# AIM-SE/AC-TSR

Measured on AMD Instinct MI355X. Metric: user-sequences/sec fwd+bwd, AC-SASRec L=50 d=64, 1/2/4/8 MI355X, higher is better.
Workload: dtype f32; 1 GPU; ACSASRec full training step (spatial + adversarial calibrators, BASELINE configs[2]), synthetic 100000-item catalogue, B=512/GPU L=50 d=64 h=2 2 layers inner=256, CE loss, two-pass backward + Adam; global_batch=512, seq_len=50, hidden=64, heads=2, parallelism=dp1, launch=hipGraph replay per step, backward=two walks (reference protocol, trainer.py:672-686)

## Files before the change

ac_tsr_amd/_lib.py:

```python
from __future__ import annotations

import ctypes as C
import os
import subprocess

_HERE = os.path.dirname(os.path.abspath(__file__))
CSRC = os.path.join(_HERE, "csrc")
LIB_PATH = os.environ.get("ACATTN_LIB") or os.path.join(CSRC, "libacattn.so")
HEADER_PATH = os.path.join(os.path.dirname(_HERE), "include", "acattn.h")

ABI_VERSION = 30
MAX_MASKS = 8
NSTAT = 8
MASK_STRUCTURED, MASK_DENSE_LL, MASK_DENSE_L = 0, 1, 2
COMBINE = {"fixed": 0, "gate": 1, "annealing": 2}
RICH = {"none": 0, "fixed": 1, "trainable": 2}
RNG_EXPLICIT, RNG_COUNTER = 0, 1
FWD_AUTO, FWD_STREAM, FWD_STAGED, FWD_GENERAL = 0, 1, 2, 3
BWD_AUTO, BWD_STREAM, BWD_ROW = 0, 1, 2

_f = C.c_void_p


class Problem(C.Structure):
    _fields_ = [
        ("B", C.c_int32), ("L", C.c_int32), ("H", C.c_int32), ("n_heads", C.c_int32),
# ... 60 lines not shown

ADAM_MAX_TENSORS = 64


class AdamGroup(C.Structure):
    _fields_ = [("n_tensors", C.c_int32), ("param", _f * ADAM_MAX_TENSORS), ("grad", _f * ADAM_MAX_TENSORS),
                ("exp_avg", _f * ADAM_MAX_TENSORS), ("exp_avg_sq", _f * ADAM_MAX_TENSORS), ("step", _f * ADAM_MAX_TENSORS),
                ("numel", C.c_int64 * ADAM_MAX_TENSORS)]


class TailProblem(C.Structure):
    _fields_ = [("rows", C.c_int32), ("H", C.c_int32), ("I", C.c_int32), ("ctx", _f), ("x", _f), ("wd", _f), ("bd", _f),
                ("g1", _f), ("b1", _f), ("w1", _f), ("bb1", _f), ("w2", _f), ("bb2", _f), ("g2", _f), ("b2", _f),
                ("eps1", C.c_float), ("eps2", C.c_float), ("p1", C.c_float), ("p2", C.c_float), ("keep1", _f),
                ("keep2", _f), ("seed1", C.c_uint64), ("seed2", C.c_uint64), ("seed_device", _f), ("src_index", _f),
                ("src_R", C.c_int32), ("src_L", C.c_int32)]


class TailSaved(C.Structure):
    _fields_ = [("h1", _f), ("st1", _f), ("a", _f), ("act", _f), ("h3", _f), ("st2", _f), ("out", _f),
                ("gelu_grad", _f)]


class TailBwdIO(C.Structure):
    _fields_ = [("d_out", _f), ("d_ctx", _f), ("d_x", _f), ("d_h1", _f), ("d_h2", _f), ("d_h3", _f), ("dgb_part", _f),
                ("workspace", _f)]


class EmbedProblem(C.Structure):
    _fields_ = [("rows", C.c_int32), ("L", C.c_int32), ("H", C.c_int32), ("n_table_rows", C.c_int64), ("idx", _f),
                ("table", _f), ("pos", _f), ("gamma", _f), ("beta", _f), ("eps", C.c_float), ("p_drop", C.c_float),
# ... 24 lines not shown
    "acattn_dropout_add_layernorm_fwd": (C.c_int, [C.POINTER(LnProblem), _f, _f, C.c_void_p]),
    "acattn_dropout_add_layernorm_bwd": (C.c_int, [C.POINTER(LnProblem), _f, _f, _f, _f, _f, C.c_void_p]),
    "acattn_embed_layernorm_fwd": (C.c_int, [C.POINTER(EmbedProblem), _f, _f, C.c_void_p]),
    "acattn_embed_layernorm_bwd": (C.c_int, [C.POINTER(EmbedProblem), _f, _f, C.c_int64, _f, _f, _f, C.c_void_p]),
    "acattn_projections_supported": (C.c_int, [C.c_int32, C.c_int32]),
    "acattn_projections_bwd_workspace_bytes": (C.c_int64, [C.POINTER(ProjProblem)]),
    "acattn_projections_fwd": (C.c_int, [C.POINTER(ProjProblem), C.POINTER(ProjOut), C.c_void_p]),
    "acattn_projections_bwd": (C.c_int, [C.POINTER(ProjProblem), C.POINTER(ProjBwdIO), C.c_void_p]),
    "acattn_layer_tail_supported": (C.c_int, [C.c_int32, C.c_int32]),
    "acattn_layer_tail_fwd": (C.c_int, [C.POINTER(TailProblem), C.POINTER(TailSaved), C.c_void_p]),
    "acattn_layer_tail_bwd": (C.c_int, [C.POINTER(TailProblem), C.POINTER(TailSaved), C.POINTER(TailBwdIO), C.c_void_p]),
    "acattn_layer_tail_bwd_partial_rows": (C.c_int32, [C.c_int32]),
    "acattn_layer_tail_bwd_partial_rows_for": (C.c_int32, [C.c_int32, C.c_int32]),
    "acattn_layer_tail_bwd_workspace_bytes": (C.c_int64, [C.c_int32, C.c_int32]),
    "acattn_select_layer_tail_blocks": (C.c_int, [C.c_int]),
    "acattn_adam_step": (C.c_int, [C.POINTER(AdamGroup), C.c_double, C.c_double, C.c_double, C.c_double, C.c_double, _f,
                                   C.c_void_p]),
    "acattn_dense_ce_fwd": (C.c_int, [_f, C.c_int64, C.c_int64, _f, _f, _f, C.c_void_p]),
    "acattn_dense_ce_bwd": (C.c_int, [_f, _f, _f, _f, C.c_int64, C.c_int64, _f, C.c_void_p]),
    "acattn_step_inputs": (C.c_int, [C.POINTER(C.c_void_p), C.POINTER(C.c_void_p), C.POINTER(C.c_int64), C.c_int32, C.c_void_p,
                                     C.c_void_p, C.c_void_p, C.c_int32, C.c_void_p]),
    "acattn_sum_rows": (C.c_int, [_f, _f, C.c_int32, C.c_int32, C.c_int32, C.c_void_p]),
    "acattn_sum_rows_pair": (C.c_int, [_f, _f, C.c_int32, C.c_int32, C.c_int32, _f, _f, C.c_int32, C.c_int32, C.c_int32, C.c_void_p]),
    "acattn_mask_penalty_fwd": (C.c_int, [_f, C.c_int64, _f, _f, C.c_void_p]),
    "acattn_mask_penalty_partial": (C.c_int, [_f, C.c_int64, _f, C.c_void_p]),
    "acattn_mask_penalty_partial_multi": (C.c_int, [C.c_void_p, C.c_int32, C.c_int64, _f, C.c_void_p]),
    "acattn_mask_penalty_bwd_scaled_multi": (C.c_int, [C.c_void_p, _f, _f, C.c_float, C.c_int64, C.c_void_p, C.c_int32,
                                                       C.c_void_p]),
    "acattn_attacked_loss_finish": (C.c_int, [_f, C.c_int32, _f, C.c_int32, C.c_int64, C.c_float, _f, _f, C.c_int32,
                                              C.c_void_p]),
# ... 68 lines not shown
```

ac_tsr_amd/csrc/acattn_api.hip:

```cpp
#include <stdint.h>
#include <stdio.h>
#include <string.h>

#include <algorithm>

#include "acattn_common.h"

namespace {
thread_local char g_err[256] = "";

int fail(const char* msg) {
  snprintf(g_err, sizeof(g_err), "%s", msg);
  return -1;
}

int check_problem(const acattn_problem* p) {
  if (!p) return fail("problem is NULL");
  if (p->B < 1 || p->L < 1 || p->H < 1 || p->n_heads < 1) return fail("B, L, H, n_heads must be positive");
  if (p->H % p->n_heads != 0)
    return fail("The hidden size is not a multiple of the number of attention heads");
  const int dh = p->H / p->n_heads;
  if (dh != 16 && dh != 32 && dh != 64 && dh != 128) return fail("unsupported head size: dh must be 16, 32, 64 or 128");
  if (p->L > 208) return fail("unsupported sequence length: L must be <= 208");
  if (!p->q || !p->k || !p->v) return fail("q, k, v must be non-NULL");
// ... 223 lines not shown
  if (!io->dmq_total && !io->dmk_total && !io->dx) return fail("projections backward: nothing to compute");
  const int rc = acattn_launch_proj_bwd(*p, *io, (hipStream_t)stream);
  if (rc > 0) snprintf(g_err, sizeof(g_err), "HIP launch failed: %s", hipGetErrorString((hipError_t)rc));
  return rc;
}

static int check_tail(const acattn_tail_problem* p, const acattn_tail_saved* s) {
  if (!p || !s) return fail("problem and saved must be non-NULL");
  if (p->rows < 1) return fail("rows must be positive");
  if (!acattn_tail_supported(p->H, p->I)) return fail("layer tail: (hidden_size, inner_size) must be (64, 256), (64, 128), (128, 512), (128, 256) or (256, 1024)");
  if (!p->ctx || !p->x || !p->wd || !p->bd || !p->g1 || !p->b1 || !p->w1 || !p->bb1 || !p->w2 || !p->bb2 || !p->g2 || !p->b2)
    return fail("layer tail: inputs and parameters must be non-NULL");
  if (!(p->p1 >= 0.f && p->p1 < 1.f) || !(p->p2 >= 0.f && p->p2 < 1.f)) return fail("dropout probabilities must be in [0, 1)");
  if (!s->h1 || !s->st1 || !s->a || !s->h3 || !s->st2) return fail("layer tail: saved tensors must be non-NULL");
  if (p->src_index && (p->src_R < 1 || p->src_L < 1)) return fail("layer tail: src_index needs src_R, src_L >= 1");
  return 0;
}

int acattn_layer_tail_supported(int32_t H, int32_t I) { return acattn_tail_supported(H, I) ? 1 : 0; }

int32_t acattn_layer_tail_bwd_partial_rows(int32_t rows) { return acattn_tail_bwd_partial_rows(rows); }
int32_t acattn_layer_tail_bwd_partial_rows_for(int32_t rows, int32_t H) { return acattn_tail_bwd_partial_rows_h(rows, H); }
int64_t acattn_layer_tail_bwd_workspace_bytes(int32_t H, int32_t I) {
  return acattn_tail_supported(H, I) ? acattn_tail_bwd_ws_bytes(H, I) : -1;
}

int acattn_select_layer_tail_blocks(int nb) {
  if (nb < 0 || nb > 2) return fail("rows per wave: 0 (automatic), 1 or 2 blocks of 16");
  return acattn_select_tail_nb(nb);
}

int acattn_layer_tail_fwd(const acattn_tail_problem* p, const acattn_tail_saved* saved, void* stream) {
  if (int rc = check_tail(p, saved)) return rc;
  if (!saved->act || !saved->out) return fail("layer tail forward: act and out must be non-NULL");
  const int rc = acattn_launch_tail_fwd(*p, *saved, (hipStream_t)stream);
  if (rc > 0) snprintf(g_err, sizeof(g_err), "HIP launch failed: %s", hipGetErrorString((hipError_t)rc));
  return rc;
}

// ... 295 lines not shown
```

ac_tsr_amd/csrc/acattn_common.h:

```cpp
#pragma once
#include <hip/hip_runtime.h>
#include <stdint.h>

#include <type_traits>

#include "acattn.h"

typedef float f4 __attribute__((ext_vector_type(4)));
typedef float f4u __attribute__((ext_vector_type(4), aligned(4)));

#define ACATTN_NEG_INF (-__builtin_inff())
#define ACATTN_MASK_FILL (-10000.0f)
#define ACATTN_LOG_EPS (1e-24f)

__device__ __forceinline__ float quad_sum(float x) {
  auto r = __builtin_amdgcn_permlane16_swap(__float_as_uint(x), __float_as_uint(x), false, false);
  x = __uint_as_float(r[0]) + __uint_as_float(r[1]);
  auto s = __builtin_amdgcn_permlane32_swap(__float_as_uint(x), __float_as_uint(x), false, false);
  return __uint_as_float(s[0]) + __uint_as_float(s[1]);
}

__device__ __forceinline__ float quad_max(float x) {
  auto r = __builtin_amdgcn_permlane16_swap(__float_as_uint(x), __float_as_uint(x), false, false);
  x = fmaxf(__uint_as_float(r[0]), __uint_as_float(r[1]));
// ... 249 lines not shown
int acattn_launch_ln_bwd(const acattn_ln_problem& p, const float* dy, const float* stats, float* dz, float* dres,
                         float* dgb_part, hipStream_t stream);
int acattn_launch_sum_rows(const float* x, float* out, int batch, int R, int C, hipStream_t stream);
int acattn_launch_sum_rows_pair(const float* x1, float* out1, int batch1, int R1, int C1, const float* x2, float* out2,
                                int batch2, int R2, int C2, hipStream_t stream);
void acattn_set_error(const char* msg);
bool acattn_proj_supported(int H, int G);
int64_t acattn_proj_bwd_ws_bytes(const acattn_proj_problem& p);
int acattn_launch_proj_fwd(const acattn_proj_problem& p, const acattn_proj_out& o, hipStream_t stream);
int acattn_launch_proj_bwd(const acattn_proj_problem& p, const acattn_proj_bwd_io& io, hipStream_t stream);
bool acattn_tail_supported(int H, int I);
int acattn_tail_bwd_partial_rows(int rows);
int acattn_tail_bwd_partial_rows_h(int rows, int H);
int64_t acattn_tail_bwd_ws_bytes(int H, int I);
int acattn_select_tail_nb(int nb);
int acattn_launch_tail_fwd(const acattn_tail_problem& p, const acattn_tail_saved& s, hipStream_t stream);
int acattn_launch_tail_bwd(const acattn_tail_problem& p, const acattn_tail_saved& s, const acattn_tail_bwd_io& io,
                           hipStream_t stream);
int64_t acattn_linear_wgrad_ws_bytes(int64_t M, int K, int N);
int acattn_launch_linear_wgrad(const float* const* x, const float* const* dy, const int* K, const int* N,
                               float* const* dw, float* const* db, int n_items, int64_t M, void* ws, hipStream_t stream,
                               int* P_out = nullptr, long long* w_off_out = nullptr, long long* b_off_out = nullptr);
int acattn_launch_linear_wgrad_reduce_many(const float* const* part_w, const float* const* part_b, const int* K, const int* N,
                                           const int* P, float* const* dw, float* const* db, int n_items,
                                           const float* const* sr_x, float* const* sr_out, const int* sr_R, const int* sr_C,
                                           int n_sr, hipStream_t stream);
int acattn_launch_embed_fwd(const acattn_embed_problem& p, float* y, float* stats, hipStream_t stream);
int acattn_launch_embed_bwd(const acattn_embed_problem& p, const float* dy, const float* stats, int64_t padding_idx,
                            float* d_table, float* d_pos_part, float* dgb_part, hipStream_t stream);
int acattn_launch_penalty_fwd(const float* m, int64_t n, float* ws, float* norm, hipStream_t stream);
// ... 35 lines not shown
```

ac_tsr_amd/csrc/acattn_tail.hip:

```cpp
#include <stdlib.h>

#include <algorithm>

#include "acattn_common.h"
#include "acattn_rowops.h"
#include "acattn_wstage.h"

int acattn_tail_bwd_partial_rows(int rows);
int acattn_tail_bwd_partial_rows_h(int rows, int H);

namespace {

int g_tail_nb = getenv("ACATTN_TAIL_BLOCKS") ? atoi(getenv("ACATTN_TAIL_BLOCKS")) : 0;
bool split_slabs(int rows) {
  static const int limit = getenv("ACATTN_TAIL_SPLIT_ROWS") ? atoi(getenv("ACATTN_TAIL_SPLIT_ROWS")) : 4096;
  return g_tail_nb == 0 && rows <= limit;
}
#ifndef ACATTN_TAIL64_WAVES
#define ACATTN_TAIL64_WAVES 3
#endif
bool staged64(int rows) {
  static const bool per_wave = getenv("ACATTN_TAIL_PER_WAVE") != nullptr;
  static const int from = getenv("ACATTN_TAIL64_STAGED_ROWS") ? atoi(getenv("ACATTN_TAIL64_STAGED_ROWS")) : 32768;
  return !per_wave && g_tail_nb == 0 && rows >= from;
// ... 446 lines not shown
    for (int t = 0; t < DT; ++t)
#pragma unroll
      for (int r = 0; r < 4; ++r)
#pragma unroll
        for (int nt = 0; nt < DT; ++nt)
#pragma unroll
          for (int nb = 0; nb < NB; ++nb) dc[nb][nt] = mfma16(wdt[nt][t][r], dh1[nb][t][r], dc[nb][nt]);
#pragma unroll
    for (int nb = 0; nb < NB; ++nb)
      if (W.ok[nb])
#pragma unroll
        for (int nt = 0; nt < DT; ++nt) store_grad(IO.d_ctx + (size_t)W.src[nb] * H + 16 * nt + 4 * g, dc[nb][nt], P.src_index != nullptr);
  }
}


template <int DT, class Emit>
__device__ __forceinline__ void stream_square(const float* w, const float* bias, int c, int g, const f4 (&in)[DT], Emit&& emit) {
  constexpr int H = 16 * DT;
  f4 wbuf[2][DT], bb[2];
  auto load = [&](int nt, f4 (&dst)[DT], f4& b) {
    b = bias ? *(const f4*)(bias + 16 * nt + 4 * g) : f4{0.f, 0.f, 0.f, 0.f};
#pragma unroll
    for (int t = 0; t < DT; ++t) dst[t] = *(const f4*)(w + (size_t)(16 * nt + c) * H + 16 * t + 4 * g);
  };
  load(0, wbuf[0], bb[0]);
  static_for<DT>([&](auto k) {
    constexpr int NT = decltype(k)::value;
    if constexpr (NT + 1 < DT) load(NT + 1, wbuf[(NT + 1) & 1], bb[(NT + 1) & 1]);
    PIN_ORDER();
// ... 932 lines not shown
  if (s.gelu_grad) {
    if (split)
      hipLaunchKernelGGL((tail_wide_bwd_kernel<H, I, 4, true>), dim3(blocks), dim3(256), 0, stream, p, s, io, (const float*)ws);
    else
      hipLaunchKernelGGL((tail_wide_bwd_kernel<H, I, 1, true>), dim3(blocks), dim3(64), 0, stream, p, s, io, (const float*)ws);
  } else {
    if (split)
      hipLaunchKernelGGL((tail_wide_bwd_kernel<H, I, 4, false>), dim3(blocks), dim3(256), 0, stream, p, s, io, (const float*)ws);
    else
      hipLaunchKernelGGL((tail_wide_bwd_kernel<H, I, 1, false>), dim3(blocks), dim3(64), 0, stream, p, s, io, (const float*)ws);
  }
  }
  return (int)hipGetLastError();
}

template <int H, int I>
int launch_fwd(const acattn_tail_problem& p, const acattn_tail_saved& s, hipStream_t stream) {
  if (staged64(p.rows)) {
    const int wgs = (p.rows + 16 * NWV - 1) / (16 * NWV);
    hipLaunchKernelGGL((tail_chunked_fwd_kernel<H, I>), dim3(wgs), dim3(64 * NWV), 0, stream, p, s);
    return (int)hipGetLastError();
  }
  const int nb = rows_per_wave(p.rows) / 16;
  const int blocks = (p.rows + 16 * nb - 1) / (16 * nb);
  if (nb == 1 && split_slabs(p.rows)) {
    hipLaunchKernelGGL((tail_fwd_kernel<H, I, 1, 4>), dim3(blocks), dim3(256), 0, stream, p, s);
    return (int)hipGetLastError();
  }
  if (nb == 2)
    hipLaunchKernelGGL((tail_fwd_kernel<H, I, 2>), dim3(blocks), dim3(64), 0, stream, p, s);
  else
    hipLaunchKernelGGL((tail_fwd_kernel<H, I, 1>), dim3(blocks), dim3(64), 0, stream, p, s);
  return (int)hipGetLastError();
}

template <int H, int I>
int launch_bwd(const acattn_tail_problem& p, const acattn_tail_saved& s, const acattn_tail_bwd_io& io, hipStream_t stream) {
  if (staged64(p.rows)) {
    if (!io.workspace) {
      acattn_set_error("layer tail backward: this row count needs acattn_tail_bwd_io.workspace (acattn_layer_tail_bwd_workspace_bytes)");
      return -1;
    }
    float* ws = (float*)io.workspace;
    hipLaunchKernelGGL(tail_transpose_kernel, dim3(I / 16, I / 16, 3), dim3(256), 0, stream, p.w1, p.w2, p.wd, H, I, ws);
    const int wgs = (p.rows + 16 * NWV - 1) / (16 * NWV);
    if (s.gelu_grad)
      hipLaunchKernelGGL((tail_chunked_bwd_kernel<H, I, true>), dim3(wgs), dim3(64 * NWV), 0, stream, p, s, io, (const float*)ws);
    else
      hipLaunchKernelGGL((tail_chunked_bwd_kernel<H, I, false>), dim3(wgs), dim3(64 * NWV), 0, stream, p, s, io, (const float*)ws);
    return (int)hipGetLastError();
  }
  const int nb = rows_per_wave(p.rows) / 16;
  const int blocks = acattn_tail_bwd_partial_rows(p.rows);
  if (nb == 1 && split_slabs(p.rows)) {
    hipLaunchKernelGGL((tail_bwd_kernel<H, I, 1, 4>), dim3(blocks), dim3(256), 0, stream, p, s, io);
    return (int)hipGetLastError();
  }
  if (nb == 2)
    hipLaunchKernelGGL((tail_bwd_kernel<H, I, 2>), dim3(blocks), dim3(64), 0, stream, p, s, io);
  else
    hipLaunchKernelGGL((tail_bwd_kernel<H, I, 1>), dim3(blocks), dim3(64), 0, stream, p, s, io);
  return (int)hipGetLastError();
}

}

bool acattn_tail_supported(int H, int I) {
  return (H == 64 && (I == 256 || I == 128)) || (H == 128 && (I == 512 || I == 256)) || (H == 256 && I == 1024);
}

int acattn_tail_bwd_partial_rows(int rows) { return (rows + rows_per_wave(rows) - 1) / rows_per_wave(rows); }
int acattn_tail_bwd_partial_rows_h(int rows, int H) {
  return (H > 64 || staged64(rows)) ? (rows + 15) / 16 : acattn_tail_bwd_partial_rows(rows);
}
int64_t acattn_tail_bwd_ws_bytes(int H, int I) { return ((int64_t)2 * H * I + (int64_t)H * H) * (int64_t)sizeof(float); }

int acattn_select_tail_nb(int nb) {
  const int prev = g_tail_nb;
  g_tail_nb = nb;
  return prev;
}

int acattn_launch_tail_fwd(const acattn_tail_problem& p, const acattn_tail_saved& s, hipStream_t stream) {
  if (p.H == 64 && p.I == 256) return launch_fwd<64, 256>(p, s, stream);
  if (p.H == 64 && p.I == 128) return launch_fwd<64, 128>(p, s, stream);
  if (p.H == 128 && p.I == 512) return launch_wide_fwd<128, 512>(p, s, stream);
  if (p.H == 128 && p.I == 256) return launch_wide_fwd<128, 256>(p, s, stream);
  if (p.H == 256 && p.I == 1024) return launch_wide_fwd<256, 1024>(p, s, stream);
  acattn_set_error("layer tail: unsupported (hidden_size, inner_size)");
  return -1;
// ... 13 lines not shown
```

ac_tsr_amd/tail.py:

```python
from __future__ import annotations

import ctypes as C

import torch
import torch.nn.functional as F

from . import _lib, fused_ln, ops
from .ops import _ptr, _stream
from .state import state_of

FUSED_KERNEL = True
FUSED_MAX_HIDDEN = 128


def _tail_problem(c, x, wd, bd, g1, b1, w1, bb1, w2, bb2, g2, b2, eps1, eps2, p1, p2, k1, k2, seed1, seed2, seed_t,
                  rows=None):
    p = _lib.TailProblem()
    H, I = wd.shape[0], w1.shape[0]
    p.rows, p.H, p.I = c.numel() // H, H, I
    if rows is not None:
        p.rows, p.src_index, p.src_R, p.src_L = rows.numel(), _ptr(rows), rows.shape[-1], c.shape[-2]
    p.ctx, p.x = _ptr(c), _ptr(x)
    p.wd, p.bd, p.g1, p.b1 = _ptr(wd), _ptr(bd), _ptr(g1), _ptr(b1)
    p.w1, p.bb1, p.w2, p.bb2, p.g2, p.b2 = _ptr(w1), _ptr(bb1), _ptr(w2), _ptr(bb2), _ptr(g2), _ptr(b2)
# ... 16 lines not shown
        H, I = c.shape[-1], w1.shape[0]
        if pick is not None:
            pick = pick.contiguous()
            assert c.dim() == 3 and x.shape == c.shape and pick.dtype == torch.int64 and pick.shape[0] == c.shape[0]
            out_shape = (*pick.shape, H)
        else:
            out_shape = c.shape
        rows = 1
        for d in out_shape[:-1]:
            rows *= d
        new = lambda *shape: torch.empty(*shape, device=c.device, dtype=torch.float32)
        h1, a, h3, out = (new(*out_shape) for _ in range(4))
        st1, st2, act = new(rows, 2), new(rows, 2), new(rows, I)
        dgelu = new(rows, I) if (H > 64 and any(ctx.needs_input_grad)) else None
        p = _tail_problem(c, x, *params, eps1, eps2, p1, p2, k1, k2, seed1, seed2, seed_tensor, pick)
        sv = _lib.TailSaved()
        sv.h1, sv.st1, sv.a, sv.act, sv.h3, sv.st2, sv.out = (_ptr(t) for t in (h1, st1, a, act, h3, st2, out))
        sv.gelu_grad = _ptr(dgelu)
        _lib.check(_lib.load().acattn_layer_tail_fwd(C.byref(p), C.byref(sv), _stream()), "layer_tail_fwd")
        empty = c.new_empty(0)
        ctx.save_for_backward(c, x, h1, st1, a, act, h3, st2, *params, k1 if k1 is not None else empty,
                              k2 if k2 is not None else empty, seed_tensor if seed_tensor is not None else empty,
                              pick if pick is not None else empty, dgelu if dgelu is not None else empty)
        ctx.args = (eps1, eps2, p1, p2, k1 is not None, k2 is not None, seed1, seed2, seed_tensor is not None,
                    pick is not None)
        return out

    @staticmethod
    def backward(ctx, d_out):
        c, x, h1, st1, a, act, h3, st2 = ctx.saved_tensors[:8]
        params = ctx.saved_tensors[8:18]
        k1, k2, seed_t, pick, dgelu = ctx.saved_tensors[18:]
        eps1, eps2, p1, p2, has_k1, has_k2, seed1, seed2, has_seed_t, has_pick = ctx.args
        k1, k2, seed_t = (k1 if has_k1 else None), (k2 if has_k2 else None), (seed_t if has_seed_t else None)
        pick = pick if has_pick else None
        want_params = not ctx.state.attack_pass_only
        need_c, need_x = ctx.needs_input_grad[0], ctx.needs_input_grad[1]
        lib = _lib.load()
        rows, H, I = act.shape[0], c.shape[-1], act.shape[-1]
        new = lambda *shape: torch.empty(*shape, device=c.device, dtype=torch.float32)
        d_out = d_out.contiguous()
        p = _tail_problem(c, x, *params, eps1, eps2, p1, p2, k1, k2, seed1, seed2, seed_t, pick)
        sv = _lib.TailSaved()
        sv.h1, sv.st1, sv.a, sv.act, sv.h3, sv.st2 = (_ptr(t) for t in (h1, st1, a, act, h3, st2))
        sv.gelu_grad = _ptr(dgelu) if dgelu.numel() else None
        io = _lib.TailBwdIO()
        if pick is not None and need_c and need_x:
            d_c, d_x = torch.zeros(2, *c.shape, device=c.device, dtype=c.dtype).unbind(0)
        else:
            alloc = torch.zeros_like if pick is not None else torch.empty_like
            d_c = alloc(c) if need_c else None
            d_x = alloc(x) if need_x else None
        io.d_out, io.d_ctx, io.d_x = _ptr(d_out), _ptr(d_c), _ptr(d_x)
        d_h1 = d_h2 = d_h3 = part = None
        if want_params:
            d_h1, d_h2, d_h3 = new(rows, H), new(rows, I), new(rows, H)
            part = new(int(lib.acattn_layer_tail_bwd_partial_rows_for(rows, H)), 4 * H)
# ... 94 lines not shown
```

include/acattn.h:

```cpp
#ifndef ACATTN_H_
#define ACATTN_H_

#include <stdint.h>

#ifdef __cplusplus
extern "C" {
#endif

#define ACATTN_ABI_VERSION 30

enum {
  ACATTN_MASK_STRUCTURED = 0,
  ACATTN_MASK_DENSE_LL = 1,
  ACATTN_MASK_DENSE_L = 2
};

enum { ACATTN_COMBINE_FIXED = 0, ACATTN_COMBINE_GATE = 1, ACATTN_COMBINE_ANNEALING = 2 };

enum { ACATTN_RICH_NONE = 0, ACATTN_RICH_FIXED = 1, ACATTN_RICH_TRAINABLE = 2 };

enum {
  ACATTN_RNG_EXPLICIT = 0,
  ACATTN_RNG_COUNTER = 1
};
// ... 206 lines not shown
  const float* b1;
  const float* w1;
  const float* bb1;
  const float* w2;
  const float* bb2;
  const float* g2;
  const float* b2;
  float eps1, eps2;
  float p1, p2;
  const uint8_t* keep1;
  const uint8_t* keep2;
  uint64_t seed1, seed2;
  const uint64_t* seed_device;
  const int64_t* src_index;
  int32_t src_R, src_L;
} acattn_tail_problem;

typedef struct acattn_tail_saved {
  float* h1;
  float* st1;
  float* a;
  float* act;
  float* h3;
  float* st2;
  float* out;
  float* gelu_grad;
} acattn_tail_saved;

typedef struct acattn_tail_bwd_io {
  const float* d_out;
// ... 2 lines not shown
  float* d_h1;
  float* d_h2;
  float* d_h3;
  float* dgb_part;
  void* workspace;
} acattn_tail_bwd_io;

int acattn_layer_tail_supported(int32_t H, int32_t I);
int acattn_layer_tail_fwd(const acattn_tail_problem* p, const acattn_tail_saved* saved, void* stream);
int acattn_layer_tail_bwd(const acattn_tail_problem* p, const acattn_tail_saved* saved, const acattn_tail_bwd_io* io,
                          void* stream);
int32_t acattn_layer_tail_bwd_partial_rows(int32_t rows);
int32_t acattn_layer_tail_bwd_partial_rows_for(int32_t rows, int32_t H);
int64_t acattn_layer_tail_bwd_workspace_bytes(int32_t H, int32_t I);
int acattn_select_layer_tail_blocks(int nb);

typedef struct acattn_proj_problem {
  int32_t rows, H, G;
  const float* x;
  const float *wq, *bq;
  const float *wk, *bk;
  const float *wv, *bv;
  const float *waq, *baq;
  const float *wak, *bak;
  const float *wg, *bg;
  const float *w_order, *b_order, *w_dist, *b_dist;
  int32_t n_heads, L;
} acattn_proj_problem;

typedef struct acattn_proj_out {
// ... 76 lines not shown
```

Baseline: 483,900 user-sequences/sec.

## Pre-split tail weights into MFMA-ready bf16 planes once per forward

Adds a kernel that converts the layer-tail weights (dense, FFN up and FFN down, plus their transposes) into pre-permuted three-way split planes laid out as MFMA fragments. New split-precision forward and backward tail kernels load these planes directly instead of splitting weights in every wave. The intent is to remove repeated per-block weight conversion and strided weight loads. The cost is an extra kernel launch and a planes buffer per forward, saved for backward. The path is used only when split products are selected and rows are not on the staged path.

```diff
diff --git a/ac_tsr_amd/_lib.py b/ac_tsr_amd/_lib.py
--- a/ac_tsr_amd/_lib.py
+++ b/ac_tsr_amd/_lib.py
@@ -9,7 +9,7 @@
 LIB_PATH = os.environ.get("ACATTN_LIB") or os.path.join(CSRC, "libacattn.so")
 HEADER_PATH = os.path.join(os.path.dirname(_HERE), "include", "acattn.h")
 
-ABI_VERSION = 30
+ABI_VERSION = 31
 MAX_MASKS = 8
 NSTAT = 8
 MASK_STRUCTURED, MASK_DENSE_LL, MASK_DENSE_L = 0, 1, 2
@@ -100,7 +100,7 @@
                 ("g1", _f), ("b1", _f), ("w1", _f), ("bb1", _f), ("w2", _f), ("bb2", _f), ("g2", _f), ("b2", _f),
                 ("eps1", C.c_float), ("eps2", C.c_float), ("p1", C.c_float), ("p2", C.c_float), ("keep1", _f),
                 ("keep2", _f), ("seed1", C.c_uint64), ("seed2", C.c_uint64), ("seed_device", _f), ("src_index", _f),
-                ("src_R", C.c_int32), ("src_L", C.c_int32)]
+                ("src_R", C.c_int32), ("src_L", C.c_int32), ("split_planes", _f)]
 
 
 class TailSaved(C.Structure):
@@ -155,6 +155,8 @@
     "acattn_layer_tail_bwd_partial_rows_for": (C.c_int32, [C.c_int32, C.c_int32]),
     "acattn_layer_tail_bwd_workspace_bytes": (C.c_int64, [C.c_int32, C.c_int32]),
     "acattn_select_layer_tail_blocks": (C.c_int, [C.c_int]),
+    "acattn_layer_tail_split_bytes": (C.c_int64, [C.c_int32, C.c_int32, C.c_int32]),
+    "acattn_layer_tail_split_weights": (C.c_int, [C.POINTER(TailProblem), C.c_void_p, C.c_void_p]),
     "acattn_adam_step": (C.c_int, [C.POINTER(AdamGroup), C.c_double, C.c_double, C.c_double, C.c_double, C.c_double, _f,
                                    C.c_void_p]),
     "acattn_dense_ce_fwd": (C.c_int, [_f, C.c_int64, C.c_int64, _f, _f, _f, C.c_void_p]),
diff --git a/ac_tsr_amd/csrc/acattn_api.hip b/ac_tsr_amd/csrc/acattn_api.hip
--- a/ac_tsr_amd/csrc/acattn_api.hip
+++ b/ac_tsr_amd/csrc/acattn_api.hip
@@ -261,6 +261,8 @@
   if (!(p->p1 >= 0.f && p->p1 < 1.f) || !(p->p2 >= 0.f && p->p2 < 1.f)) return fail("dropout probabilities must be in [0, 1)");
   if (!s->h1 || !s->st1 || !s->a || !s->h3 || !s->st2) return fail("layer tail: saved tensors must be non-NULL");
   if (p->src_index && (p->src_R < 1 || p->src_L < 1)) return fail("layer tail: src_index needs src_R, src_L >= 1");
+  if (p->split_planes && p->H != 64) return fail("layer tail: split_planes is for hidden 64 only");
+  if (((uintptr_t)p->split_planes & 15) != 0) return fail("layer tail: split_planes must be 16-byte aligned");
   return 0;
 }
 
@@ -270,6 +272,19 @@
 int32_t acattn_layer_tail_bwd_partial_rows_for(int32_t rows, int32_t H) { return acattn_tail_bwd_partial_rows_h(rows, H); }
 int64_t acattn_layer_tail_bwd_workspace_bytes(int32_t H, int32_t I) {
   return acattn_tail_supported(H, I) ? acattn_tail_bwd_ws_bytes(H, I) : -1;
+}
+
+int64_t acattn_layer_tail_split_bytes(int32_t H, int32_t I, int32_t rows) {
+  return acattn_tail_supported(H, I) && rows > 0 ? acattn_tail_split_bytes(H, I, rows) : 0;
+}
+
+int acattn_layer_tail_split_weights(const acattn_tail_problem* p, void* planes, void* stream) {
+  if (!p || !planes || !p->wd || !p->w1 || !p->w2) return fail("layer tail split planes: problem, weights and planes must be non-NULL");
+  if (p->H != 64 || (p->I != 256 && p->I != 128)) return fail("layer tail split planes: hidden 64, inner 256 or 128 only");
+  if (((uintptr_t)planes & 15) != 0) return fail("layer tail split planes: planes must be 16-byte aligned");
+  const int rc = acattn_launch_tail_split(*p, planes, (hipStream_t)stream);
+  if (rc > 0) snprintf(g_err, sizeof(g_err), "HIP launch failed: %s", hipGetErrorString((hipError_t)rc));
+  return rc;
 }
 
 int acattn_select_layer_tail_blocks(int nb) {
diff --git a/ac_tsr_amd/csrc/acattn_common.h b/ac_tsr_amd/csrc/acattn_common.h
--- a/ac_tsr_amd/csrc/acattn_common.h
+++ b/ac_tsr_amd/csrc/acattn_common.h
@@ -287,6 +287,8 @@
 int acattn_tail_bwd_partial_rows_h(int rows, int H);
 int64_t acattn_tail_bwd_ws_bytes(int H, int I);
 int acattn_select_tail_nb(int nb);
+int64_t acattn_tail_split_bytes(int H, int I, int rows);
+int acattn_launch_tail_split(const acattn_tail_problem& p, void* planes, hipStream_t stream);
 int acattn_launch_tail_fwd(const acattn_tail_problem& p, const acattn_tail_saved& s, hipStream_t stream);
 int acattn_launch_tail_bwd(const acattn_tail_problem& p, const acattn_tail_saved& s, const acattn_tail_bwd_io& io,
                            hipStream_t stream);
diff --git a/ac_tsr_amd/csrc/acattn_tail.hip b/ac_tsr_amd/csrc/acattn_tail.hip
--- a/ac_tsr_amd/csrc/acattn_tail.hip
+++ b/ac_tsr_amd/csrc/acattn_tail.hip
@@ -1,9 +1,11 @@
 #include <stdlib.h>
+#include <string.h>
 
 #include <algorithm>
 
 #include "acattn_common.h"
 #include "acattn_rowops.h"
+#include "acattn_split.h"
 #include "acattn_wstage.h"
 
 int acattn_tail_bwd_partial_rows(int rows);
@@ -484,6 +486,399 @@
   }
 }
 
+
+template <int I>
+struct TailPlanes {
+  static constexpr int SQ = 64 * 64 * 3 / 8, RECT = I * 64 * 3 / 8;
+  static constexpr int FWD_D = 0, FWD_1 = SQ, FWD_2 = SQ + RECT;
+  static constexpr int BWD_D = SQ + 2 * RECT, BWD_1 = 2 * SQ + 2 * RECT, BWD_2 = 2 * SQ + 3 * RECT;
+  static constexpr int TOTAL = 2 * SQ + 4 * RECT;
+};
+
+__device__ __forceinline__ int tail_kperm(int s, int g, int j) { return 32 * s + 16 * (j >> 2) + 4 * g + (j & 3); }
+
+template <int I>
+__global__ void __launch_bounds__(256) tail_split_planes_kernel(const float* wd, const float* w1, const float* w2, b8* planes) {
+  using L = TailPlanes<I>;
+  const int mtx = blockIdx.y, which = mtx % 3;
+  const bool T = mtx >= 3;
+  const float* w = which == 0 ? wd : which == 1 ? w1 : w2;
+  const int M = which == 0 ? 64 : ((which == 1) != T ? I : 64), K = (which == 0 ? 64 * 64 : 64 * I) / M, KS = K / 32;
+  b8* dst = planes + (mtx == 0 ? L::FWD_D : mtx == 1 ? L::FWD_1 : mtx == 2 ? L::FWD_2 : mtx == 3 ? L::BWD_D : mtx == 4 ? L::BWD_1 : L::BWD_2);
+  const int idx = blockIdx.x * 256 + threadIdx.x;
+  if (idx >= (M / 16) * KS * 64) return;
+  const int lane = idx & 63, f = idx >> 6, mt = f / KS, s = f % KS, c = lane & 15, g = lane >> 4, m = 16 * mt + c;
+  float x[8];
+#pragma unroll
+  for (int j = 0; j < 8; ++j) {
+    const int k = tail_kperm(s, g, j);
+    x[j] = T ? w[(size_t)k * M + m] : w[(size_t)m * K + k];
+  }
+  b8 p[3];
+  split8(x, p[0], p[1], p[2]);
+#pragma unroll
+  for (int q = 0; q < 3; ++q) dst[((size_t)f * 3 + q) * 64 + lane] = p[q];
+}
+
+template <int KS>
+__device__ __forceinline__ void load_frag(const b8* mat, int mt, int s, int lane, b8 (&a)[3]) {
+#pragma unroll
+  for (int q = 0; q < 3; ++q) a[q] = mat[((mt * KS + s) * 3 + q) * 64 + lane];
+}
+
+__device__ __forceinline__ void split_tiles(const f4 lo, const f4 hi, b8 (&b)[3]) {
+  float x[8];
+#pragma unroll
+  for (int r = 0; r < 4; ++r) {
+    x[r] = lo[r];
+    x[4 + r] = hi[r];
+  }
+  split8(x, b[0], b[1], b[2]);
+}
+
+template <int NB>
+__device__ __forceinline__ void split_rows64(const f4 (&v)[NB][4], b8 (&b)[NB][2][3]) {
+#pragma unroll
+  for (int nb = 0; nb < NB; ++nb)
+#pragma unroll
+    for (int s = 0; s < 2; ++s) split_tiles(v[nb][2 * s], v[nb][2 * s + 1], b[nb][s]);
+}
+
+template <int NB>
+__device__ __forceinline__ void split_square(const b8* mat, int lane, const b8 (&b)[NB][2][3], f4 (&acc)[NB][4]) {
+#pragma unroll
+  for (int nt = 0; nt < 4; ++nt)
+#pragma unroll
+    for (int s = 0; s < 2; ++s) {
+      b8 w[3];
+      load_frag<2>(mat, nt, s, lane, w);
+#pragma unroll
+      for (int nb = 0; nb < NB; ++nb) acc[nb][nt] = mfma_split(w, b[nb][s], acc[nb][nt]);
+    }
+}
+
+template <int H, int I, int NB, int NW = 1>
+__global__ void __launch_bounds__(64 * NW) tail_split_fwd_kernel(const acattn_tail_problem P, const acattn_tail_saved S) {
+  static_assert(H == 64 && (NW == 1 || NB == 1), "hidden 64; the slab split works on one row block");
+  using L = TailPlanes<I>;
+  constexpr int DT = 4, NP = I / 32, NJ = NP / NW;
+  static_assert(NP % NW == 0 && NJ >= 1, "whole pairs per wave");
+  const int lane = threadIdx.x & 63, c = lane & 15, g = lane >> 4;
+  const int wave = NW > 1 ? __builtin_amdgcn_readfirstlane(threadIdx.x >> 6) : 0;
+  const Rows<NB> W = wave_rows<NB>(P);
+  const uint64_t step = P.seed_device ? *P.seed_device : 0ull;
+  const b8* planes = (const b8*)P.split_planes;
+  const b8 *pw1 = planes + L::FWD_1, *pw2 = planes + L::FWD_2;
+
+  struct W1Pair {
+    b8 w[2][2][3];
+    f4 b[2];
+  };
+  auto load_w1 = [&](int p, W1Pair& d) {
+#pragma unroll
+    for (int tt = 0; tt < 2; ++tt) {
+#pragma unroll
+      for (int s = 0; s < 2; ++s) load_frag<2>(pw1, 2 * p + tt, s, lane, d.w[tt][s]);
+      d.b[tt] = *(const f4*)(P.bb1 + 32 * p + 16 * tt + 4 * g);
+    }
+  };
+  W1Pair w1b[2];
+  load_w1(wave, w1b[0]);
+
+  f4 h1[NB][DT], a[NB][DT];
+  {
+    f4 cb[NB][DT], res[NB][DT], bd[DT], g1[DT], b1[DT];
+#pragma unroll
+    for (int nb = 0; nb < NB; ++nb)
+#pragma unroll
+      for (int t = 0; t < DT; ++t) {
+        cb[nb][t] = *(const f4*)(P.ctx + (size_t)W.src[nb] * H + 16 * t + 4 * g);
+        res[nb][t] = *(const f4*)(P.x + (size_t)W.src[nb] * H + 16 * t + 4 * g);
+      }
+    load_cols<DT>(P.bd, g, bd);
+    load_cols<DT>(P.g1, g, g1);
+    load_cols<DT>(P.b1, g, b1);
+    b8 cs[NB][2][3];
+    split_rows64<NB>(cb, cs);
+#pragma unroll
+    for (int nb = 0; nb < NB; ++nb)
+#pragma unroll
+      for (int nt = 0; nt < DT; ++nt) h1[nb][nt] = bd[nt];
+    split_square<NB>(planes + L::FWD_D, lane, cs, h1);
+#pragma unroll
+    for (int nb = 0; nb < NB; ++nb) {
+      f4 keep[DT];
+#pragma unroll
+      for (int t = 0; t < DT; ++t) keep[t] = row_keep_scale(P.p1, P.keep1, P.seed1 + step, W.row[nb], 4 * t + g, H);
+      float mean, rstd;
+      ln_forward<DT>(h1[nb], res[nb], keep, g1, b1, P.eps1, a[nb], mean, rstd);
+      if (W.ok[nb] && wave == 0) {
+#pragma unroll
+        for (int t = 0; t < DT; ++t) {
+          const size_t o = (size_t)W.row[nb] * H + 16 * t + 4 * g;
+          *(f4*)(S.h1 + o) = h1[nb][t];
+          *(f4*)(S.a + o) = a[nb][t];
+        }
+        if (g == 0) *(float2*)(S.st1 + 2 * (size_t)W.row[nb]) = float2{mean, rstd};
+      }
+    }
+  }
+
+  b8 as[NB][2][3];
+  split_rows64<NB>(a, as);
+  f4 h3[NB][DT];
+#pragma unroll
+  for (int nt = 0; nt < DT; ++nt) {
+    const f4 bb2 = *(const f4*)(P.bb2 + 16 * nt + 4 * g);
+#pragma unroll
+    for (int nb = 0; nb < NB; ++nb) h3[nb][nt] = wave == 0 ? bb2 : f4{0.f, 0.f, 0.f, 0.f};
+  }
+  static_for<NJ>([&](auto jc) {
+    constexpr int J = decltype(jc)::value;
+    const int p = wave + NW * J;
+    b8 w2[DT][3];
+#pragma unroll
+    for (int nt = 0; nt < DT; ++nt) load_frag<NP>(pw2, nt, p, lane, w2[nt]);
+    if constexpr (J + 1 < NJ) load_w1(p + NW, w1b[(J + 1) & 1]);
+    PIN_ORDER();
+    const W1Pair& cur = w1b[J & 1];
+    f4 h2[NB][2];
+#pragma unroll
+    for (int tt = 0; tt < 2; ++tt)
+#pragma unroll
+      for (int nb = 0; nb < NB; ++nb) h2[nb][tt] = f4{0.f, 0.f, 0.f, 0.f};
+#pragma unroll
+    for (int tt = 0; tt < 2; ++tt)
+#pragma unroll
+      for (int s = 0; s < 2; ++s)
+#pragma unroll
+        for (int nb = 0; nb < NB; ++nb) h2[nb][tt] = mfma_split(cur.w[tt][s], as[nb][s], h2[nb][tt]);
+#pragma unroll
+    for (int nb = 0; nb < NB; ++nb) {
+      f4 act[2];
+#pragma unroll
+      for (int tt = 0; tt < 2; ++tt) {
+        const f4 pre = h2[nb][tt] + cur.b[tt];
+#pragma unroll
+        for (int r = 0; r < 4; ++r) act[tt][r] = gelu_erf(pre[r]);
+        if (W.ok[nb]) *(f4*)(S.act + (size_t)W.row[nb] * I + 32 * p + 16 * tt + 4 * g) = act[tt];
+      }
+      b8 ap[3];
+      split_tiles(act[0], act[1], ap);
+#pragma unroll
+      for (int nt = 0; nt < DT; ++nt) h3[nb][nt] = mfma_split(w2[nt], ap, h3[nb][nt]);
+    }
+    PIN_ORDER();
+  });
+
+  if (NW > 1) {
+    __shared__ f4 red[NW > 1 ? NW - 1 : 1][DT][64];
+    if (wave > 0) {
+#pragma unroll
+      for (int t = 0; t < DT; ++t) red[wave - 1][t][lane] = h3[0][t];
+    }
+    __syncthreads();
+    if (wave > 0) return;
+#pragma unroll
+    for (int w = 0; w < NW - 1; ++w)
+#pragma unroll
+      for (int t = 0; t < DT; ++t) h3[0][t] += red[w][t][lane];
+  }
+
+  f4 g2[DT], b2[DT];
+  load_cols<DT>(P.g2, g, g2);
+  load_cols<DT>(P.b2, g, b2);
+#pragma unroll
+  for (int nb = 0; nb < NB; ++nb) {
+    f4 keep[DT], y[DT];
+#pragma unroll
+    for (int t = 0; t < DT; ++t) keep[t] = row_keep_scale(P.p2, P.keep2, P.seed2 + step, W.row[nb], 4 * t + g, H);
+    float mean, rstd;
+    ln_forward<DT>(h3[nb], a[nb], keep, g2, b2, P.eps2, y, mean, rstd);
+    if (W.ok[nb]) {
+#pragma unroll
+      for (int t = 0; t < DT; ++t) {
+        const size_t o = (size_t)W.row[nb] * H + 16 * t + 4 * g;
+        *(f4*)(S.h3 + o) = h3[nb][t];
+        *(f4*)(S.out + o) = y[t];
+      }
+      if (g == 0) *(float2*)(S.st2 + 2 * (size_t)W.row[nb]) = float2{mean, rstd};
+    }
+  }
+}
+
+template <int H, int I, int NB, int NW = 1>
+__global__ void __launch_bounds__(64 * NW) tail_split_bwd_kernel(const acattn_tail_problem P, const acattn_tail_saved S,
+                                                                 const acattn_tail_bwd_io IO) {
+  static_assert(H == 64 && (NW == 1 || NB == 1), "hidden 64; the slab split works on one row block");
+  using L = TailPlanes<I>;
+  constexpr int DT = 4, NP = I / 32, NJ = NP / NW;
+  static_assert(NP % NW == 0 && NJ >= 1, "whole pairs per wave");
+  const int lane = threadIdx.x & 63, c = lane & 15, g = lane >> 4;
+  const int wave = NW > 1 ? __builtin_amdgcn_readfirstlane(threadIdx.x >> 6) : 0;
+  const Rows<NB> W = wave_rows<NB>(P);
+  const uint64_t step = P.seed_device ? *P.seed_device : 0ull;
+  float* part = IO.dgb_part ? IO.dgb_part + (size_t)blockIdx.x * 4 * H : nullptr;
+  const b8* planes = (const b8*)P.split_planes;
+  const b8 *pw1 = planes + L::FWD_1, *pw1t = planes + L::BWD_1, *pw2t = planes + L::BWD_2;
+
+  struct Pair {
+    b8 w1[2][2][3], w2t[2][2][3];
+    f4 b[2];
+  };
+  auto load_pair = [&](int p, Pair& d) {
+#pragma unroll
+    for (int tt = 0; tt < 2; ++tt) {
+#pragma unroll
+      for (int s = 0; s < 2; ++s) {
+        load_frag<2>(pw1, 2 * p + tt, s, lane, d.w1[tt][s]);
+        load_frag<2>(pw2t, 2 * p + tt, s, lane, d.w2t[tt][s]);
+      }
+      d.b[tt] = *(const f4*)(P.bb1 + 32 * p + 16 * tt + 4 * g);
+    }
+  };
+  Pair pb[2];
+  load_pair(wave, pb[0]);
+
+  f4 a[NB][DT], dh3[NB][DT], da[NB][DT];
+  {
+    f4 acc_g[DT], acc_b[DT];
+#pragma unroll
+    for (int t = 0; t < DT; ++t) acc_g[t] = acc_b[t] = f4{0.f, 0.f, 0.f, 0.f};
+#pragma unroll
+    for (int nb = 0; nb < NB; ++nb) {
+      f4 z[DT], keep[DT], dy[DT];
+#pragma unroll
+      for (int t = 0; t < DT; ++t) {
+        const size_t o = (size_t)W.row[nb] * H + 16 * t + 4 * g;
+        z[t] = *(const f4*)(S.h3 + o);
+        a[nb][t] = *(const f4*)(S.a + o);
+        dy[t] = *(const f4*)(IO.d_out + o);
+        keep[t] = row_keep_scale(P.p2, P.keep2, P.seed2 + step, W.row[nb], 4 * t + g, H);
+      }
+      const float2 st = *(const float2*)(S.st2 + 2 * (size_t)W.row[nb]);
+      ln_backward<DT>(z, a[nb], keep, P.g2, st.x, st.y, dy, W.ok[nb], g, da[nb], acc_g, acc_b);
+#pragma unroll
+      for (int t = 0; t < DT; ++t) {
+        dh3[nb][t] = da[nb][t] * keep[t];
+        if (IO.d_h3 && W.ok[nb] && wave == 0) *(f4*)(IO.d_h3 + (size_t)W.row[nb] * H + 16 * t + 4 * g) = dh3[nb][t];
+        if (wave > 0) da[nb][t] = f4{0.f, 0.f, 0.f, 0.f};
+      }
+    }
+    if (part && wave == 0) {
+      store_partial<DT>(part + 2 * H, acc_g, c, g);
+      store_partial<DT>(part + 3 * H, acc_b, c, g);
+    }
+  }
+
+  {
+    b8 as[NB][2][3], ds[NB][2][3];
+    split_rows64<NB>(a, as);
+    split_rows64<NB>(dh3, ds);
+    static_for<NJ>([&](auto jc) {
+      constexpr int J = decltype(jc)::value;
+      const int p = wave + NW * J;
+      b8 w1t[DT][3];
+#pragma unroll
+      for (int nt = 0; nt < DT; ++nt) load_frag<NP>(pw1t, nt, p, lane, w1t[nt]);
+      if constexpr (J + 1 < NJ) load_pair(p + NW, pb[(J + 1) & 1]);
+      PIN_ORDER();
+      const Pair& cur = pb[J & 1];
+      f4 h2[NB][2], dact[NB][2];
+#pragma unroll
+      for (int tt = 0; tt < 2; ++tt)
+#pragma unroll
+        for (int nb = 0; nb < NB; ++nb) h2[nb][tt] = dact[nb][tt] = f4{0.f, 0.f, 0.f, 0.f};
+#pragma unroll
+      for (int tt = 0; tt < 2; ++tt)
+#pragma unroll
+        for (int s = 0; s < 2; ++s)
+#pragma unroll
+          for (int nb = 0; nb < NB; ++nb) {
+            h2[nb][tt] = mfma_split(cur.w1[tt][s], as[nb][s], h2[nb][tt]);
+            dact[nb][tt] = mfma_split(cur.w2t[tt][s], ds[nb][s], dact[nb][tt]);
+          }
+#pragma unroll
+      for (int nb = 0; nb < NB; ++nb) {
+        f4 dh2[2];
+#pragma unroll
+        for (int tt = 0; tt < 2; ++tt) {
+          const f4 pre = h2[nb][tt] + cur.b[tt];
+#pragma unroll
+          for (int r = 0; r < 4; ++r) dh2[tt][r] = dact[nb][tt][r] * gelu_erf_grad(pre[r]);
+          if (IO.d_h2 && W.ok[nb]) *(f4*)(IO.d_h2 + (size_t)W.row[nb] * I + 32 * p + 16 * tt + 4 * g) = dh2[tt];
+        }
+        b8 dp[3];
+        split_tiles(dh2[0], dh2[1], dp);
+#pragma unroll
+        for (int nt = 0; nt < DT; ++nt) da[nb][nt] = mfma_split(w1t[nt], dp, da[nb][nt]);
+      }
+      PIN_ORDER();
+    });
+  }
+
+  if (NW > 1) {
+    __shared__ f4 red[NW > 1 ? NW - 1 : 1][DT][64];
+    if (wave > 0) {
+#pragma unroll
+      for (int t = 0; t < DT; ++t) red[wave - 1][t][lane] = da[0][t];
+    }
+    __syncthreads();
+    if (wave > 0) return;
+#pragma unroll
+    for (int w = 0; w < NW - 1; ++w)
+#pragma unroll
+      for (int t = 0; t < DT; ++t) da[0][t] += red[w][t][lane];
+  }
+
+  f4 dh1[NB][DT];
+  {
+    f4 acc_g[DT], acc_b[DT];
+#pragma unroll
+    for (int t = 0; t < DT; ++t) acc_g[t] = acc_b[t] = f4{0.f, 0.f, 0.f, 0.f};
+#pragma unroll
+    for (int nb = 0; nb < NB; ++nb) {
+      f4 z[DT], res[DT], keep[DT], dz[DT];
+#pragma unroll
+      for (int t = 0; t < DT; ++t) {
+        const size_t o = (size_t)W.row[nb] * H + 16 * t + 4 * g;
+        z[t] = *(const f4*)(S.h1 + o);
+        res[t] = *(const f4*)(P.x + (size_t)W.src[nb] * H + 16 * t + 4 * g);
+        keep[t] = row_keep_scale(P.p1, P.keep1, P.seed1 + step, W.row[nb], 4 * t + g, H);
+      }
+      const float2 st = *(const float2*)(S.st1 + 2 * (size_t)W.row[nb]);
+      ln_backward<DT>(z, res, keep, P.g1, st.x, st.y, da[nb], W.ok[nb], g, dz, acc_g, acc_b);
+#pragma unroll
+      for (int t = 0; t < DT; ++t) {
+        const size_t o = (size_t)W.row[nb] * H + 16 * t + 4 * g;
+        dh1[nb][t] = dz[t] * keep[t];
+        if (W.ok[nb]) {
+          if (IO.d_x) store_grad(IO.d_x + (size_t)W.src[nb] * H + 16 * t + 4 * g, dz[t], P.src_index != nullptr);
+          if (IO.d_h1) *(f4*)(IO.d_h1 + o) = dh1[nb][t];
+        }
+      }
+    }
+    if (part) {
+      store_partial<DT>(part, acc_g, c, g);
+      store_partial<DT>(part + H, acc_b, c, g);
+    }
+  }
+  if (IO.d_ctx) {
+    f4 dc[NB][DT];
+#pragma unroll
+    for (int nb = 0; nb < NB; ++nb)
+#pragma unroll
+      for (int nt = 0; nt < DT; ++nt) dc[nb][nt] = f4{0.f, 0.f, 0.f, 0.f};
+    b8 hs[NB][2][3];
+    split_rows64<NB>(dh1, hs);
+    split_square<NB>(planes + L::BWD_D, lane, hs, dc);
+#pragma unroll
+    for (int nb = 0; nb < NB; ++nb)
+      if (W.ok[nb])
+#pragma unroll
+        for (int nt = 0; nt < DT; ++nt) store_grad(IO.d_ctx + (size_t)W.src[nb] * H + 16 * nt + 4 * g, dc[nb][nt], P.src_index != nullptr);
+  }
+}
 
 template <int DT, class Emit>
 __device__ __forceinline__ void stream_square(const float* w, const float* bias, int c, int g, const f4 (&in)[DT], Emit&& emit) {
@@ -1446,6 +1841,18 @@
   return (int)hipGetLastError();
 }
 
+bool tail_split_products(int H, int I, int rows) {
+  static const char* e = getenv("ACATTN_TAIL_PRODUCTS");
+  static const bool fp32 = e && !strcmp(e, "fp32");
+  return H == 64 && (I == 256 || I == 128) && !fp32 && acattn_linear_products_choice(-1) == 1 && !staged64(rows);
+}
+
+template <int I>
+int launch_split_planes(const acattn_tail_problem& p, void* planes, hipStream_t stream) {
+  hipLaunchKernelGGL(tail_split_planes_kernel<I>, dim3(I / 32, 6), dim3(256), 0, stream, p.wd, p.w1, p.w2, (b8*)planes);
+  return (int)hipGetLastError();
+}
+
 template <int H, int I>
 int launch_fwd(const acattn_tail_problem& p, const acattn_tail_saved& s, hipStream_t stream) {
   if (staged64(p.rows)) {
@@ -1455,6 +1862,15 @@
   }
   const int nb = rows_per_wave(p.rows) / 16;
   const int blocks = (p.rows + 16 * nb - 1) / (16 * nb);
+  if (p.split_planes) {
+    if (nb == 1 && split_slabs(p.rows))
+      hipLaunchKernelGGL((tail_split_fwd_kernel<H, I, 1, 4>), dim3(blocks), dim3(256), 0, stream, p, s);
+    else if (nb == 2)
+      hipLaunchKernelGGL((tail_split_fwd_kernel<H, I, 2>), dim3(blocks), dim3(64), 0, stream, p, s);
+    else
+      hipLaunchKernelGGL((tail_split_fwd_kernel<H, I, 1>), dim3(blocks), dim3(64), 0, stream, p, s);
+    return (int)hipGetLastError();
+  }
   if (nb == 1 && split_slabs(p.rows)) {
     hipLaunchKernelGGL((tail_fwd_kernel<H, I, 1, 4>), dim3(blocks), dim3(256), 0, stream, p, s);
     return (int)hipGetLastError();
@@ -1484,6 +1900,13 @@
   }
   const int nb = rows_per_wave(p.rows) / 16;
   const int blocks = acattn_tail_bwd_partial_rows(p.rows);
+  if (p.split_planes && !(nb == 1 && split_slabs(p.rows))) {
+    if (nb == 2)
+      hipLaunchKernelGGL((tail_split_bwd_kernel<H, I, 2>), dim3(blocks), dim3(64), 0, stream, p, s, io);
+    else
+      hipLaunchKernelGGL((tail_split_bwd_kernel<H, I, 1>), dim3(blocks), dim3(64), 0, stream, p, s, io);
+    return (int)hipGetLastError();
+  }
   if (nb == 1 && split_slabs(p.rows)) {
     hipLaunchKernelGGL((tail_bwd_kernel<H, I, 1, 4>), dim3(blocks), dim3(256), 0, stream, p, s, io);
     return (int)hipGetLastError();
@@ -1506,6 +1929,18 @@
   return (H > 64 || staged64(rows)) ? (rows + 15) / 16 : acattn_tail_bwd_partial_rows(rows);
 }
 int64_t acattn_tail_bwd_ws_bytes(int H, int I) { return ((int64_t)2 * H * I + (int64_t)H * H) * (int64_t)sizeof(float); }
+
+int64_t acattn_tail_split_bytes(int H, int I, int rows) {
+  if (!tail_split_products(H, I, rows)) return 0;
+  return (int64_t)(I == 256 ? TailPlanes<256>::TOTAL : TailPlanes<128>::TOTAL) * (int64_t)sizeof(b8);
+}
+
+int acattn_launch_tail_split(const acattn_tail_problem& p, void* planes, hipStream_t stream) {
+  if (p.H == 64 && p.I == 256) return launch_split_planes<256>(p, planes, stream);
+  if (p.H == 64 && p.I == 128) return launch_split_planes<128>(p, planes, stream);
+  acattn_set_error("layer tail split planes: hidden 64, inner 256 or 128 only");
+  return -1;
+}
 
 int acattn_select_tail_nb(int nb) {
   const int prev = g_tail_nb;
diff --git a/ac_tsr_amd/tail.py b/ac_tsr_amd/tail.py
--- a/ac_tsr_amd/tail.py
+++ b/ac_tsr_amd/tail.py
@@ -54,14 +54,22 @@
         st1, st2, act = new(rows, 2), new(rows, 2), new(rows, I)
         dgelu = new(rows, I) if (H > 64 and any(ctx.needs_input_grad)) else None
         p = _tail_problem(c, x, *params, eps1, eps2, p1, p2, k1, k2, seed1, seed2, seed_tensor, pick)
+        lib = _lib.load()
+        planes = None
+        nbytes = int(lib.acattn_layer_tail_split_bytes(H, I, rows))
+        if nbytes > 0:
+            planes = new(nbytes // 4)
+            _lib.check(lib.acattn_layer_tail_split_weights(C.byref(p), _ptr(planes), _stream()), "layer_tail_split_weights")
+            p.split_planes = _ptr(planes)
         sv = _lib.TailSaved()
         sv.h1, sv.st1, sv.a, sv.act, sv.h3, sv.st2, sv.out = (_ptr(t) for t in (h1, st1, a, act, h3, st2, out))
         sv.gelu_grad = _ptr(dgelu)
-        _lib.check(_lib.load().acattn_layer_tail_fwd(C.byref(p), C.byref(sv), _stream()), "layer_tail_fwd")
+        _lib.check(lib.acattn_layer_tail_fwd(C.byref(p), C.byref(sv), _stream()), "layer_tail_fwd")
         empty = c.new_empty(0)
         ctx.save_for_backward(c, x, h1, st1, a, act, h3, st2, *params, k1 if k1 is not None else empty,
                               k2 if k2 is not None else empty, seed_tensor if seed_tensor is not None else empty,
-                              pick if pick is not None else empty, dgelu if dgelu is not None else empty)
+                              pick if pick is not None else empty, dgelu if dgelu is not None else empty,
+                              planes if planes is not None else empty)
         ctx.args = (eps1, eps2, p1, p2, k1 is not None, k2 is not None, seed1, seed2, seed_tensor is not None,
                     pick is not None)
         return out
@@ -70,7 +78,7 @@
     def backward(ctx, d_out):
         c, x, h1, st1, a, act, h3, st2 = ctx.saved_tensors[:8]
         params = ctx.saved_tensors[8:18]
-        k1, k2, seed_t, pick, dgelu = ctx.saved_tensors[18:]
+        k1, k2, seed_t, pick, dgelu, planes = ctx.saved_tensors[18:]
         eps1, eps2, p1, p2, has_k1, has_k2, seed1, seed2, has_seed_t, has_pick = ctx.args
         k1, k2, seed_t = (k1 if has_k1 else None), (k2 if has_k2 else None), (seed_t if has_seed_t else None)
         pick = pick if has_pick else None
@@ -81,6 +89,7 @@
         new = lambda *shape: torch.empty(*shape, device=c.device, dtype=torch.float32)
         d_out = d_out.contiguous()
         p = _tail_problem(c, x, *params, eps1, eps2, p1, p2, k1, k2, seed1, seed2, seed_t, pick)
+        p.split_planes = _ptr(planes) if planes.numel() else None
         sv = _lib.TailSaved()
         sv.h1, sv.st1, sv.a, sv.act, sv.h3, sv.st2 = (_ptr(t) for t in (h1, st1, a, act, h3, st2))
         sv.gelu_grad = _ptr(dgelu) if dgelu.numel() else None
diff --git a/include/acattn.h b/include/acattn.h
--- a/include/acattn.h
+++ b/include/acattn.h
@@ -7,7 +7,7 @@
 extern "C" {
 #endif
 
-#define ACATTN_ABI_VERSION 30
+#define ACATTN_ABI_VERSION 31
 
 enum {
   ACATTN_MASK_STRUCTURED = 0,
@@ -244,6 +244,7 @@
   const uint64_t* seed_device;
   const int64_t* src_index;
   int32_t src_R, src_L;
+  const void* split_planes;
 } acattn_tail_problem;
 
 typedef struct acattn_tail_saved {
@@ -276,6 +277,8 @@
 int32_t acattn_layer_tail_bwd_partial_rows_for(int32_t rows, int32_t H);
 int64_t acattn_layer_tail_bwd_workspace_bytes(int32_t H, int32_t I);
 int acattn_select_layer_tail_blocks(int nb);
+int64_t acattn_layer_tail_split_bytes(int32_t H, int32_t I, int32_t rows);
+int acattn_layer_tail_split_weights(const acattn_tail_problem* p, void* planes, void* stream);
 
 typedef struct acattn_proj_problem {
   int32_t rows, H, G;
```

After: 492,500 user-sequences/sec, median of 6. +1.8%, better.
